# second-state/qwen3_asr_rs

Hardware: AMD Instinct MI355X
Metric: audio-seconds/sec (RTFx) Qwen3-ASR-0.6B greedy, 30s clips (higher is better)
Workload: dtype bf16; 1 GPU; Qwen3-ASR-0.6b bf16, batch=1 x 30s synthetic 16kHz clip per GPU, 100 new tokens (fixed, EOS ignored); clips_per_gpu=1, parallelism=dp1 (independent utterances per GPU, no data-path collective)

## Files before the change

### qwen3_asr_rs_amd/csrc/k_gemv.hip

```cpp
#include <algorithm>
#include <type_traits>

#include "argmax.h"


namespace q3a {

int gemv_rows_per_wave(const GemvArgs& a) {
  const int logical = (a.mode == 2) ? a.N / 2 : a.N;
  if (logical >= 32768 && a.K <= 2048) return 4;
  if (logical >= 4096 || a.mode == 2) return 2;
  return 1;
}
int gemv_blocks(const GemvArgs& a) {
  const int pr = gemv_rows_per_wave(a);
  const int rows_per_wave = (a.mode == 2) ? pr / 2 : pr;
  const int logical = (a.mode == 2) ? a.N / 2 : a.N;
  return (logical + 4 * rows_per_wave - 1) / (4 * rows_per_wave);
}

namespace {

constexpr int ATTN_F_MAX = 1024;
struct AttnTables {
// ... 90 lines not shown
    M = Mn;
  }
  const float inv = 1.0f / L;
#pragma unroll
  for (int e = 0; e < 8; ++e) x[e] *= inv;
}

template <int PR>
__device__ __forceinline__ void gemv_rows(const GemvArgs& a, int g, int (&prow)[PR]) {
#pragma unroll
  for (int i = 0; i < PR; ++i) {
    if (a.mode == 2) {
      const int j = g * (PR / 2) + (i >> 1);
      prow[i] = (j / 16) * 32 + (j % 16) + ((i & 1) ? 16 : 0);
    } else {
      prow[i] = g * PR + i;
    }
    if (prow[i] >= a.N) prow[i] = -1;
  }
}

__device__ __forceinline__ float dot8(const uint4& w, const float (&x)[8], float s) {
  f32x2_t a = f32x2_t{bf16lo(w.x), bf16hi(w.x)} * f32x2_t{x[0], x[1]};
  a += f32x2_t{bf16lo(w.y), bf16hi(w.y)} * f32x2_t{x[2], x[3]};
  a += f32x2_t{bf16lo(w.z), bf16hi(w.z)} * f32x2_t{x[4], x[5]};
  a += f32x2_t{bf16lo(w.w), bf16hi(w.w)} * f32x2_t{x[6], x[7]};
  return s + (a.x + a.y);
}

__device__ __forceinline__ uint4 ld_w16(const GemvArgs& a, int prow, int k) {
  const int row = prow >= 0 ? prow : a.N - 1;
  return ld_stream16(a.W + (size_t)row * a.K + k);
}
template <int KI, int PR>
__device__ __forceinline__ void request_rows(const GemvArgs& a, const int (&prow)[PR], const int (&kk)[KI], uint4 (&wq)[KI][PR]) {
#pragma unroll
  for (int it = 0; it < KI; ++it)
#pragma unroll
    for (int i = 0; i < PR; ++i) wq[it][i] = ld_w16(a, prow[i], kk[it]);
}
template <int KI>
__device__ __forceinline__ void lane_cols(int lane, int K, bool (&kin)[KI], int (&kk)[KI]) {
#pragma unroll
  for (int it = 0; it < KI; ++it) {
    const int k = lane * 8 + it * 512;
    kin[it] = k < K;
    kk[it] = kin[it] ? k : 0;
  }
}
template <int KI>
__device__ __forceinline__ void fetch_cols(const GemvArgs& a, const int (&kk)[KI], float4 (&xr)[KI][2], float4 (&nr)[KI][2]) {
#pragma unroll
  for (int it = 0; it < KI; ++it) {
    xr[it][0] = *reinterpret_cast<const float4*>(a.x + kk[it]);
    xr[it][1] = *reinterpret_cast<const float4*>(a.x + kk[it] + 4);
    nr[it][0] = *reinterpret_cast<const float4*>(a.rms_w + kk[it]);
    nr[it][1] = *reinterpret_cast<const float4*>(a.rms_w + kk[it] + 4);
  }
}
template <int KI, bool YY = false>
__device__ __forceinline__ void unpack_cols(int K, const bool (&kin)[KI], const float4 (&xr)[KI][2], const float4 (&nr)[KI][2],
                                            float (&x)[KI][8], float& ss, float* yy = nullptr) {
#pragma unroll
  for (int it = 0; it < KI; ++it) {
    const float4 v0 = xr[it][0], v1 = xr[it][1];
    const float xv[8] = {v0.x, v0.y, v0.z, v0.w, v1.x, v1.y, v1.z, v1.w};
#pragma unroll
    for (int e = 0; e < 8; ++e) x[it][e] = (K == KI * 512 || kin[it]) ? xv[e] : 0.f;
    const float4 w0 = nr[it][0], w1 = nr[it][1];
    const float wv[8] = {w0.x, w0.y, w0.z, w0.w, w1.x, w1.y, w1.z, w1.w};
#pragma unroll
    for (int e = 0; e < 8; ++e) { ss += x[it][e] * x[it][e]; x[it][e] *= wv[e]; }
    if constexpr (YY) {
#pragma unroll
      for (int e = 0; e < 8; ++e) *yy += x[it][e] * x[it][e];
    }
  }
}
template <bool LP, int NB>
__device__ __forceinline__ ArgmaxAcc<LP> merge_wave_partials(float (*am_v)[NB], int (*am_i)[NB], float (*am_s)[NB], int b) {
  ArgmaxAcc<LP> r{am_v[0][b], am_i[0][b], LP ? am_s[0][b] : 0.f};
  for (int w = 1; w < 4; ++w) r.merge(am_v[w][b], am_i[w][b], LP ? am_s[w][b] : 0.f);
  return r;
}

template <int NB, int PR, bool LP>
__device__ __forceinline__ void gemv_epilogue(const GemvArgs& a, int g, const int (&prow)[PR], float (&acc)[PR][NB],
                                              float (*am_v)[NB], int (*am_i)[NB], float (*am_s)[NB]) {
  const int tid = threadIdx.x, lane = tid & 63, wave = tid >> 6;
  if (a.mode == 3) {
    ArgmaxAcc<LP> m[NB];
    float lv[LP ? PR : 1][NB];
#pragma unroll
    for (int i = 0; i < PR; ++i) {
      if constexpr (LP) {
#pragma unroll
        for (int b = 0; b < NB; ++b) lv[i][b] = -INFINITY;
      }
      if (prow[i] < 0) continue;
#pragma unroll
      for (int b = 0; b < NB; ++b) {
        float v = acc[i][b];
        if (a.bias) v += a.bias[prow[i]];
        if (lane == 0 && a.out) a.out[(size_t)b * a.ldo + prow[i]] = v;
        if (v > m[b].v) { m[b].v = v; m[b].i = prow[i]; }
        if constexpr (LP) lv[i][b] = v;
      }
    }
    if (lane == 0) {
#pragma unroll
      for (int b = 0; b < NB; ++b) {
        am_v[wave][b] = m[b].v; am_i[wave][b] = m[b].i;
        if constexpr (LP) {
          float ws = 0.f;
#pragma unroll
          for (int i = 0; i < PR; ++i) ws += lse_term(1.f, lv[i][b], m[b].v);
          am_s[wave][b] = ws;
        }
      }
    }
    __syncthreads();
    if (tid < NB) merge_wave_partials<LP, NB>(am_v, am_i, am_s, tid).store(a.part, tid, g >> 2);
    return;
  }
  if (lane != 0) return;
  if (a.mode != 2) {
#pragma unroll
    for (int i = 0; i < PR; ++i) {
      if (prow[i] < 0) continue;
      const int n = prow[i];
#pragma unroll
      for (int b = 0; b < NB; ++b) {
        float v = acc[i][b];
        if (a.bias) v += a.bias[n];
        if (a.mode == 1) v += a.resid[(size_t)b * a.ldo + n];
        a.out[(size_t)b * a.ldo + n] = v;
      }
    }
  } else {
#pragma unroll
    for (int i = 0; i + 1 < PR; i += 2) {
      if (prow[i] < 0) continue;
      const int j = g * (PR / 2) + (i >> 1);
#pragma unroll
      for (int b = 0; b < NB; ++b) {
        float gv = acc[i][b], uv = acc[i + 1][b];
        if (a.bias) { gv += a.bias[prow[i]]; uv += a.bias[prow[i + 1]]; }
        a.out[(size_t)b * a.ldo + j] = silu_sel(gv, a.fast_math != 0) * uv;
      }
    }
  }
}

template <int PR, int KI, bool RMS, bool ATTN, int MF, bool XL, bool XP = false>
__device__ __forceinline__ void gemv1_body(const GemvArgs& a) {
  static_assert(!XL || !ATTN, "the merged attention vector already goes through LDS");
  static_assert(!XP || (XL && RMS), "the partial vectors are added in the hand-over of the norm-fused XL form");
  constexpr bool XH = !RMS && !ATTN && KI > 4;
  constexpr bool XLDS = XL || XH;
  static_assert(!XH || KI % 2 == 0, "the hand-over stores unguarded: its rounds of 1024 columns must end at KI * 512");
  __shared__ __attribute__((aligned(16))) float x_lds[(ATTN || XLDS) ? KI * 512 : 4], xl_w[(XL && RMS) ? KI * 512 : 4];
  const int tid = threadIdx.x, lane = tid & 63, wave = tid >> 6;
  Q3A_STAMP_ENTRY(t_entry);
  const int K = a.K;
  const int g = blockIdx.x * 4 + wave;
  int prow[PR];
  gemv_rows<PR>(a, g, prow);
  bool kin[KI];
  int kk[KI];
#pragma unroll
  for (int it = 0; it < KI; ++it) {
    const int k = lane * 8 + it * 512;
    kin[it] = k < K;
    kk[it] = kin[it] ? k : 0;
  }
  float4 xr[KI][2], nr[RMS ? KI : 1][2];
  uint4 wq[KI][PR];
  constexpr int XLN = (KI + 1) / 2;
  float4 xl_rx[XLDS ? XLN : 1], xl_rw[(XL && RMS) ? XLN : 1];
  constexpr int XPN = XP ? GEMV_X_PARTS_MAX : 1;
  float4 xp_r[XP ? XLN : 1][XPN];
  auto request_x = [&]() {
    if (ATTN) return;
    if constexpr (XLDS) {
#pragma unroll
      for (int j = 0; j < XLN; ++j) {
        const int k = (tid + j * 256) * 4, kc = k < K ? k : 0;
        xl_rx[j] = *reinterpret_cast<const float4*>(a.x + kc);
        if constexpr (XP) {
#pragma unroll
          for (int h = 0; h < XPN; ++h)
            xp_r[j][h] = *reinterpret_cast<const float4*>(a.x_parts + (size_t)(h < a.x_nparts ? h : a.x_nparts - 1) * K + kc);
        }
        if (RMS) xl_rw[j] = *reinterpret_cast<const float4*>(a.rms_w + kc);
      }
      return;
    }
#pragma unroll
    for (int it = 0; it < KI; ++it) {
      xr[it][0] = *reinterpret_cast<const float4*>(a.x + kk[it]);
      xr[it][1] = *reinterpret_cast<const float4*>(a.x + kk[it] + 4);
      if (RMS) {
        nr[it][0] = *reinterpret_cast<const float4*>(a.rms_w + kk[it]);
        nr[it][1] = *reinterpret_cast<const float4*>(a.rms_w + kk[it] + 4);
      }
    }
  };
  auto request_w = [&]() {
#pragma unroll
    for (int it = 0; it < KI; ++it)
#pragma unroll
      for (int i = 0; i < PR; ++i) {
        const int row = prow[i] >= 0 ? prow[i] : a.N - 1;
        wq[it][i] = ld_stream16(a.W + (size_t)row * K + kk[it]);
      }
  };
  constexpr int MCH = MF > 0 ? MF : 1;
  float mg_m[MCH], mg_l[MCH];
  float4 mg_o0[MCH], mg_o1[MCH];
  const int mg_k = lane * 8 + wave * 512;
  const bool mg_on = wave < KI && mg_k < K;
  if constexpr (ATTN && MF > 0) {
    const int kc = mg_k < K ? mg_k : 0;
    const int h = kc >> 7, d = kc & 127, ns = a.attn_nsplit, base = h * ns;
    typedef float __attribute__((ext_vector_type(4), aligned(4))) f4u_t;
#pragma unroll
    for (int j = 0; j < MCH; j += 4) {
      const f4u_t m4 = *reinterpret_cast<const f4u_t*>(a.attn_pm + base + j), l4 = *reinterpret_cast<const f4u_t*>(a.attn_pl + base + j);
#pragma unroll
      for (int e = 0; e < 4; ++e) {
        mg_m[j + e] = j + e < ns ? m4[e] : -INFINITY;
        mg_l[j + e] = j + e < ns ? l4[e] : 0.f;
      }
    }
#pragma unroll
    for (int j = 0; j < MCH; ++j) attn_partial_row8(a, base, j, d, mg_o0[j], mg_o1[j]);
    __builtin_amdgcn_sched_barrier(0);
  }
  if (RMS || XLDS) { request_x(); request_w(); } else { request_w(); request_x(); }
  if constexpr (ATTN && MF > 0) __builtin_amdgcn_sched_barrier(0);
  float bv[PR], rv[PR];
#pragma unroll
  for (int i = 0; i < PR; ++i) {
    const int n = prow[i] >= 0 ? prow[i] : 0;
    bv[i] = a.bias ? a.bias[n] : 0.f;
    rv[i] = a.mode == 1 ? a.resid[n] : 0.f;
  }
  __builtin_amdgcn_sched_barrier(0);
  Q3A_STAMP_AT(a.stamp, blockIdx.x, 1);
  Q3A_STAMP_PUT(a.stamp, blockIdx.x, 0, t_entry);
  Q3A_ARG(a.out); Q3A_ARG(a.fast_math);
  if (ATTN) Q3A_ARG(a.attn_fast_exp);
  if constexpr (ATTN && MF > 0) {
    if (mg_on) {
      const bool fast = a.attn_fast_exp != 0;
      float Mn = -INFINITY;
#pragma unroll
      for (int j = 0; j < MCH; ++j) Mn = fmaxf(Mn, mg_m[j]);
      float L = 0.f, v[8];
#pragma unroll
      for (int e = 0; e < 8; ++e) v[e] = 0.f;
#pragma unroll
      for (int j = 0; j < MCH; ++j) {
        const float f = fast ? __expf(mg_m[j] - Mn) : expf(mg_m[j] - Mn);
        L += mg_l[j] * f;
        v[0] += mg_o0[j].x * f; v[1] += mg_o0[j].y * f; v[2] += mg_o0[j].z * f; v[3] += mg_o0[j].w * f;
        v[4] += mg_o1[j].x * f; v[5] += mg_o1[j].y * f; v[6] += mg_o1[j].z * f; v[7] += mg_o1[j].w * f;
      }
      const float inv = 1.0f / L;
#pragma unroll
      for (int e = 0; e < 8; ++e) v[e] *= inv;
      *reinterpret_cast<float4*>(x_lds + mg_k) = make_float4(v[0], v[1], v[2], v[3]);
      *reinterpret_cast<float4*>(x_lds + mg_k + 4) = make_float4(v[4], v[5], v[6], v[7]);
    }
    __syncthreads();
  } else if constexpr (ATTN) {
    auto merge_pieces = [&](auto fast_c, auto ch_c) {
#pragma unroll
      for (int it = 0; it < KI; ++it) {
        if ((it & 3) == wave && kin[it]) {
          float v[8];
          attn_merge8_ch<decltype(fast_c)::value, decltype(ch_c)::value>(a, 0, kk[it], v);
          *reinterpret_cast<float4*>(x_lds + kk[it]) = make_float4(v[0], v[1], v[2], v[3]);
          *reinterpret_cast<float4*>(x_lds + kk[it] + 4) = make_float4(v[4], v[5], v[6], v[7]);
        }
      }
    };
    typedef std::integral_constant<int, 4> Ch4;
    typedef std::integral_constant<int, 8> Ch8;
    if (a.attn_fast_exp) {
      if (a.attn_nsplit <= 4) merge_pieces(std::true_type{}, Ch4{}); else merge_pieces(std::true_type{}, Ch8{});
    } else {
      if (a.attn_nsplit <= 4) merge_pieces(std::false_type{}, Ch4{}); else merge_pieces(std::false_type{}, Ch8{});
    }
    __syncthreads();
  }
  if constexpr (XLDS) {
#pragma unroll
    for (int j = 0; j < XLN; ++j) {
      const int k = (tid + j * 256) * 4;
      if (XH || k < KI * 512) {
        float4 v = xl_rx[j];
        if constexpr (XP) {
#pragma unroll
          for (int h = 0; h < XPN; ++h)
            if (h < a.x_nparts) { v.x += xp_r[j][h].x; v.y += xp_r[j][h].y; v.z += xp_r[j][h].z; v.w += xp_r[j][h].w; }
          if (blockIdx.x == 0 && k < K) *reinterpret_cast<float4*>(a.x_out + k) = v;
        }
        *reinterpret_cast<float4*>(x_lds + k) = make_float4(v.x, v.y, v.z, v.w);
        if (RMS) *reinterpret_cast<float4*>(xl_w + k) = xl_rw[j];
      }
    }
    __syncthreads();
  }
  if constexpr (ATTN || XLDS) {
#pragma unroll
    for (int it = 0; it < KI; ++it) {
      xr[it][0] = *reinterpret_cast<const float4*>(x_lds + kk[it]);
      xr[it][1] = *reinterpret_cast<const float4*>(x_lds + kk[it] + 4);
      if (XL && RMS) {
        nr[it][0] = *reinterpret_cast<const float4*>(xl_w + kk[it]);
        nr[it][1] = *reinterpret_cast<const float4*>(xl_w + kk[it] + 4);
      }
    }
  }
  Q3A_STAMP_AT(a.stamp, blockIdx.x, 2);
  float x[KI][8], acc[PR];
  float ss = 0.f;
#pragma unroll
  for (int it = 0; it < KI; ++it) {
    const float4 v0 = xr[it][0], v1 = xr[it][1];
    const float xv[8] = {v0.x, v0.y, v0.z, v0.w, v1.x, v1.y, v1.z, v1.w};
#pragma unroll
    for (int e = 0; e < 8; ++e) x[it][e] = (K == KI * 512 || kin[it]) ? xv[e] : 0.f;
    if (RMS) {
      const float4 w0 = nr[it][0], w1 = nr[it][1];
      const float wv[8] = {w0.x, w0.y, w0.z, w0.w, w1.x, w1.y, w1.z, w1.w};
#pragma unroll
      for (int e = 0; e < 8; ++e) { ss += x[it][e] * x[it][e]; x[it][e] *= wv[e]; }
    }
  }
#pragma unroll
  for (int i = 0; i < PR; ++i) acc[i] = 0.f;
#pragma unroll
  for (int it = 0; it < KI; ++it)
#pragma unroll
    for (int i = 0; i < PR; ++i) acc[i] = dot8(wq[it][i], x[it], acc[i]);
  if (wave == 0) asm volatile("" ::"v"(acc[0]));
  Q3A_STAMP_AT(a.stamp, blockIdx.x, 3);
  float rstd = 1.0f;
  if (RMS) rstd = rstd_of(wave_sum_fast(ss) / (float)K + a.eps, a.fast_math != 0);
#pragma unroll
  for (int i = 0; i < PR; ++i) acc[i] = wave_sum_fast(acc[i]) * rstd + bv[i];
  if (lane != 0) return;
  if (a.mode != 2) {
#pragma unroll
    for (int i = 0; i < PR; ++i)
      if (prow[i] >= 0) a.out[prow[i]] = acc[i] + rv[i];
  } else {
#pragma unroll
    for (int i = 0; i + 1 < PR; i += 2)
      if (prow[i] >= 0) a.out[g * (PR / 2) + (i >> 1)] = silu_sel(acc[i], a.fast_math != 0) * acc[i + 1];
  }
  Q3A_STAMP_AT(a.stamp, blockIdx.x, 4);
}

struct GemvTail {
  float* out; int fast_math;
  Q3A_STAMP_FIELD
};
struct GemvAttnTail {
  float* out; const float* bias; int attn_heads; int attn_fast_exp; int fast_math;
  Q3A_STAMP_FIELD
};
#ifdef Q3A_STAMP
#define Q3A_STAMP_COPY(dst, src) (dst).stamp = (src).stamp
#else
#define Q3A_STAMP_COPY(dst, src) do { } while (0)
#endif
template <int PR, int KI, bool RMS, bool ATTN, int MF = 0, bool XL = false>
__global__ __launch_bounds__(256) void gemv1_kernel(const uint16_t* W, const float* x, const float* rms_w, const float* bias,
                                                    const float* resid, int N, int K, int mode, float eps, GemvTail t) {
  static_assert(!ATTN, "the ATTN forms take the partials in their head");
  GemvArgs a{};
  a.W = W; a.x = x; a.rms_w = rms_w; a.bias = bias; a.resid = resid; a.N = N; a.K = K; a.mode = mode; a.eps = eps;
  a.out = t.out; a.fast_math = t.fast_math;
  Q3A_STAMP_COPY(a, t);
  gemv1_body<PR, KI, RMS, ATTN, MF, XL>(a);
}
template <int PR, int KI, bool RMS, bool ATTN, int MF = 0, bool XL = false>
__global__ __launch_bounds__(256) void gemv1_kernel(const float* attn_pm, const float* attn_pl, const float* attn_po, const uint16_t* W,
                                                    const float* resid, int N, int K, int attn_nsplit, int mode, GemvAttnTail t) {
  static_assert(ATTN && !RMS, "the plain forms take x and the norm weight in their head");
  GemvArgs a{};
  a.attn_pm = attn_pm; a.attn_pl = attn_pl; a.attn_po = attn_po; a.W = W; a.resid = resid; a.N = N; a.K = K; a.attn_nsplit = attn_nsplit;
  a.mode = mode;
  a.out = t.out; a.bias = t.bias; a.attn_heads = t.attn_heads; a.attn_fast_exp = t.attn_fast_exp; a.fast_math = t.fast_math;
  Q3A_STAMP_COPY(a, t);
  gemv1_body<PR, KI, RMS, ATTN, MF, XL>(a);
}

struct GemvXpTail {
  float* out; float* x_out; int fast_math;
  Q3A_STAMP_FIELD
};
template <int PR, int KI>
__global__ __launch_bounds__(256) void gemv1_xp_kernel(const uint16_t* W, const float* x, const float* rms_w, const float* x_parts,
                                                       const float* bias, int N, int K, int x_nparts, float eps, GemvXpTail t) {
  GemvArgs a{};
  a.W = W; a.x = x; a.rms_w = rms_w; a.x_parts = x_parts; a.bias = bias; a.N = N; a.K = K; a.x_nparts = x_nparts; a.eps = eps; a.mode = 2;
  a.out = t.out; a.x_out = t.x_out; a.fast_math = t.fast_math;
  Q3A_STAMP_COPY(a, t);
  gemv1_body<PR, KI, true, false, 0, true, true>(a);
}

struct OprojHeadTail {
  const float* bias;
  Q3A_STAMP_FIELD
};
template <int CW, int RB>
__global__ __launch_bounds__(256) void oproj_head_kernel(const float* pm, const float* pl, const float* po, const uint16_t* W, float* y_part,
                                                         int N, int K, int nsplit, int n_parts, OprojHeadTail t) {
  constexpr int NS = OPROJ_HEAD_MAX_SPLITS;
  constexpr int HEADS = CW / 128;
  constexpr int LPR = CW / 8;
  constexpr int RPI = 64 / LPR;
  constexpr int NI = RB / 4 / RPI;
  constexpr int E4 = CW / 4;
  constexpr int TG = 256 / E4;
  constexpr int SPT = NS / TG;
  static_assert(CW == 128 || CW == 256 || CW == 512, "a slice is 1, 2 or 4 q heads");
  static_assert(NI >= 1 && NI * RPI * 4 == RB && SPT * TG == NS && HEADS * NS <= 256, "row block / split plan");
  __shared__ float m_s[HEADS * NS], l_s[HEADS * NS], inv_s[HEADS];
  __shared__ __attribute__((aligned(16))) float red[TG][CW];
  const int tid = threadIdx.x, lane = tid & 63, wave = tid >> 6;
  Q3A_STAMP_ENTRY(t_entry);
  const int part = blockIdx.x % n_parts, rb = blockIdx.x / n_parts;
  const int q0 = part * HEADS;
  const int e4 = tid % E4, tg = tid / E4, hh = e4 >> 5, d = (e4 & 31) * 4;
  const int st = tid < HEADS * NS ? tid : HEADS * NS - 1, st_j = st % NS, st_jc = st_j < nsplit ? st_j : nsplit - 1;
  float st_m = pm[(size_t)(q0 + st / NS) * nsplit + st_jc], st_l = pl[(size_t)(q0 + st / NS) * nsplit + st_jc];
  float4 o[SPT];
#pragma unroll
  for (int i = 0; i < SPT; ++i) {
    const int j = tg + i * TG, jc = j < nsplit ? j : nsplit - 1;
    o[i] = *reinterpret_cast<const float4*>(po + ((size_t)(q0 + hh) * nsplit + jc) * 128 + d);
  }
  __builtin_amdgcn_sched_barrier(0);
  const int row0 = rb * RB + wave * (RB / 4) + lane / LPR;
  uint4 wq[NI];
#pragma unroll
  for (int i = 0; i < NI; ++i) {
    const int row = row0 + i * RPI, rc = row < N ? row : N - 1;
    wq[i] = ld_stream16(W + (size_t)rc * K + part * CW + (lane % LPR) * 8);
  }
  __builtin_amdgcn_sched_barrier(0);
  float bv[NI];
#pragma unroll
  for (int i = 0; i < NI; ++i) {
    const int row = row0 + i * RPI;
    bv[i] = (t.bias && part == 0) ? t.bias[row < N ? row : N - 1] : 0.f;
  }
  __builtin_amdgcn_sched_barrier(0);
  Q3A_STAMP_AT(t.stamp, blockIdx.x, 1);
  Q3A_STAMP_PUT(t.stamp, blockIdx.x, 0, t_entry);
  if (st_j >= nsplit) { st_m = -INFINITY; st_l = 0.f; }
  if (tid < HEADS * NS) { m_s[tid] = st_m; l_s[tid] = st_l; }
  __syncthreads();
  float M = -INFINITY, L = 0.f;
#pragma unroll
  for (int j = 0; j < NS; ++j) M = fmaxf(M, m_s[hh * NS + j]);
#pragma unroll
  for (int j = 0; j < NS; ++j) L += l_s[hh * NS + j] * __expf(m_s[hh * NS + j] - M);
  float4 acc = make_float4(0.f, 0.f, 0.f, 0.f);
#pragma unroll
  for (int i = 0; i < SPT; ++i) {
    const float f = __expf(m_s[hh * NS + tg + i * TG] - M);
    acc.x += o[i].x * f; acc.y += o[i].y * f; acc.z += o[i].z * f; acc.w += o[i].w * f;
  }
  *reinterpret_cast<float4*>(&red[tg][e4 * 4]) = acc;
  if (tg == 0 && (e4 & 31) == 0) inv_s[hh] = 1.0f / L;
  __syncthreads();
  const int c0 = (lane % LPR) * 8;
  float x[8];
#pragma unroll
  for (int e = 0; e < 8; ++e) x[e] = 0.f;
#pragma unroll
  for (int g = 0; g < TG; ++g) {
    const float4 a0 = *reinterpret_cast<const float4*>(&red[g][c0]), a1 = *reinterpret_cast<const float4*>(&red[g][c0 + 4]);
    x[0] += a0.x; x[1] += a0.y; x[2] += a0.z; x[3] += a0.w; x[4] += a1.x; x[5] += a1.y; x[6] += a1.z; x[7] += a1.w;
  }
  const float inv = inv_s[c0 >> 7];
#pragma unroll
  for (int e = 0; e < 8; ++e) x[e] *= inv;
  Q3A_STAMP_AT(t.stamp, blockIdx.x, 2);
  float y[NI];
#pragma unroll
  for (int i = 0; i < NI; ++i) {
    float v = row16_sum(dot8(wq[i], x, 0.f));
    if (LPR >= 32) v = xor16_sum(v);
    if (LPR >= 64) v = xor32_sum(v);
    y[i] = v + bv[i];
  }
  if (wave == 0) asm volatile("" ::"v"(y[0]));
  Q3A_STAMP_AT(t.stamp, blockIdx.x, 3);
  if (lane % LPR == 0) {
#pragma unroll
    for (int i = 0; i < NI; ++i) {
      const int row = row0 + i * RPI;
      if (row < N) y_part[(size_t)part * N + row] = y[i];
    }
  }
  Q3A_STAMP_AT(t.stamp, blockIdx.x, 4);
}

template <int PR, int KI, bool LP = false>
__device__ __forceinline__ void gemv1_head_block(const GemvArgs& a, int blk, float (&am_v)[4][1], int (&am_i)[4][1], float (*am_s)[1],
                                                 ArgmaxAcc<LP>& out) {
  const int tid = threadIdx.x, lane = tid & 63, wave = tid >> 6;
  const int g = blk * 4 + wave;
  int prow[PR];
  gemv_rows<PR>(a, g, prow);
  bool kin[KI];
  int kk[KI];
  lane_cols<KI>(lane, a.K, kin, kk);
  float4 xr[KI][2], nr[KI][2];
  uint4 wq[KI][PR];
  fetch_cols<KI>(a, kk, xr, nr);
  request_rows<KI, PR>(a, prow, kk, wq);
  float bv[PR];
#pragma unroll
  for (int i = 0; i < PR; ++i) bv[i] = a.bias ? a.bias[prow[i] >= 0 ? prow[i] : 0] : 0.f;
  __builtin_amdgcn_sched_barrier(0);
  float x[KI][8], acc[PR];
  float ss = 0.f;
  unpack_cols<KI>(a.K, kin, xr, nr, x, ss);
#pragma unroll
  for (int i = 0; i < PR; ++i) acc[i] = 0.f;
#pragma unroll
  for (int it = 0; it < KI; ++it)
#pragma unroll
    for (int i = 0; i < PR; ++i) acc[i] = dot8(wq[it][i], x[it], acc[i]);
  const float rstd = rstd_of(wave_sum_fast(ss) / (float)a.K + a.eps, a.fast_math != 0);
#pragma unroll
  for (int i = 0; i < PR; ++i) acc[i] = wave_sum_fast(acc[i]) * rstd + bv[i];
  ArgmaxAcc<LP> m;
#pragma unroll
  for (int i = 0; i < PR; ++i) {
    if (prow[i] < 0) continue;
    if (lane == 0 && a.out) a.out[prow[i]] = acc[i];
    if (acc[i] > m.v) { m.v = acc[i]; m.i = prow[i]; }
  }
  if (lane == 0) { am_v[wave][0] = m.v; am_i[wave][0] = m.i; }
  if constexpr (LP) {
    float ws = 0.f;
#pragma unroll
    for (int i = 0; i < PR; ++i) ws += prow[i] < 0 ? 0.f : lse_term(1.f, acc[i], m.v);
    if (lane == 0) am_s[wave][0] = ws;
  }
  __syncthreads();
  if (tid == 0) out = merge_wave_partials<LP, 1>(am_v, am_i, am_s, 0);
}

template <int PR, int KI, bool LP = false>
__global__ __launch_bounds__(256) void gemv1_head_kernel(const uint16_t* W, const float* x, const float* rms_w, const float* bias, float* out,
                                                         int N, int K, float eps, int fast_math, ArgmaxPartials part) {
// ... 184 lines not shown
    if (i < nb) t = fmaxf(t, v.x);
    if (i + 1 < nb) t = fmaxf(t, v.y);
    if (i + 2 < nb) t = fmaxf(t, v.z);
    if (i + 3 < nb) t = fmaxf(t, v.w);
  };
#pragma unroll
  for (int j = 0; j < PRE; ++j) fold(lv[j], tid + j * 256);
  for (int i4 = tid + PRE * 256; i4 < n4; i4 += 256) fold(lo4[i4], i4);
  t = wave_max(t);
  if (lane == 0) red[wave] = t;
  cand[tid] = 0;
  __syncthreads();
  const float T = fmaxf(fmaxf(red[0], red[1]), fmaxf(red[2], red[3]));
  if (mb < nb) cand[tid] = !(hv < T);
  __syncthreads();
  const int nj = (nb - blockIdx.x + G - 1) / G;
  ArgmaxAcc<false> best;
  int nc = 0;
  for (int j = 0; j < nj; ++j) {
    if (!cand[j]) continue;
    ArgmaxAcc<false> r;
    gemv1_head_block<PR, KI>(g, blockIdx.x + j * G, am_v, am_i, nullptr, r);
    if (tid == 0) best.merge(r);
    ++nc;
    __syncthreads();
  }
  if (tid == 0) {
    best.store(g.part, 0, blockIdx.x);
    if (tl.stats) {
      if (nc) atomicAdd(&tl.stats[0], nc);
      if (blockIdx.x == 0) atomicAdd(&tl.stats[1], 1);
    }
  }
}

template <int NB, int PR, int PF, bool LP = false>
__global__ __launch_bounds__(256) void gemvn_kernel(GemvArgs a) {
  extern __shared__ __attribute__((aligned(16))) float xs[];
  __shared__ float red[NB][4];
  __shared__ float am_v[4][NB];
  __shared__ int am_i[4][NB];
  __shared__ float am_s[LP ? 4 : 1][NB];
  const int tid = threadIdx.x, lane = tid & 63, wave = tid >> 6;
  const int K = a.K;
  const int g = blockIdx.x * 4 + wave;
  int prow[PR];
  gemv_rows<PR>(a, g, prow);
  bool kin[PF];
  int kk[PF];
  lane_cols<PF>(lane, K, kin, kk);
  uint4 wq[PF][PR];
  request_rows<PF, PR>(a, prow, kk, wq);
  __shared__ AttnTables f_s;
  if (a.attn_po) attn_scales(a, NB, f_s);
#pragma unroll
  for (int b = 0; b < NB; ++b) {
    float ss = 0.f;
    for (int k = tid * 8; k < K; k += 2048) {
      float x[8];
      if (a.attn_po) {
        attn_combined8(a, b, k, f_s, x);
      } else {
        const float4 v0 = *reinterpret_cast<const float4*>(a.x + (size_t)b * a.ldx + k);
        const float4 v1 = *reinterpret_cast<const float4*>(a.x + (size_t)b * a.ldx + k + 4);
        x[0] = v0.x; x[1] = v0.y; x[2] = v0.z; x[3] = v0.w; x[4] = v1.x; x[5] = v1.y; x[6] = v1.z; x[7] = v1.w;
      }
      if (a.rms_w) {
        const float4 w0 = *reinterpret_cast<const float4*>(a.rms_w + k);
        const float4 w1 = *reinterpret_cast<const float4*>(a.rms_w + k + 4);
        const float wv[8] = {w0.x, w0.y, w0.z, w0.w, w1.x, w1.y, w1.z, w1.w};
#pragma unroll
        for (int e = 0; e < 8; ++e) { ss += x[e] * x[e]; x[e] *= wv[e]; }
      }
      *reinterpret_cast<float4*>(xs + (size_t)b * K + k) = make_float4(x[0], x[1], x[2], x[3]);
      *reinterpret_cast<float4*>(xs + (size_t)b * K + k + 4) = make_float4(x[4], x[5], x[6], x[7]);
    }
    if (a.rms_w) {
      ss = wave_sum_fast(ss);
      if (lane == 0) red[b][wave] = ss;
    }
  }
  __syncthreads();
  float acc[PR][NB];
#pragma unroll
  for (int i = 0; i < PR; ++i)
#pragma unroll
    for (int b = 0; b < NB; ++b) acc[i][b] = 0.f;
  auto fma_all = [&](const uint4 (&w)[PR], int k) {
#pragma unroll
    for (int b = 0; b < NB; ++b) {
      const float4 xa = *reinterpret_cast<const float4*>(xs + (size_t)b * K + k);
      const float4 xb = *reinterpret_cast<const float4*>(xs + (size_t)b * K + k + 4);
      const float x[8] = {xa.x, xa.y, xa.z, xa.w, xb.x, xb.y, xb.z, xb.w};
#pragma unroll
      for (int i = 0; i < PR; ++i) acc[i][b] = dot8(w[i], x, acc[i][b]);
    }
  };
#pragma unroll
  for (int it = 0; it < PF; ++it)
    if (kin[it]) fma_all(wq[it], kk[it]);
  for (int k = lane * 8 + PF * 512; k < K; k += 512) {
    uint4 w[PR];
#pragma unroll
    for (int i = 0; i < PR; ++i) w[i] = ld_w16(a, prow[i], k);
    fma_all(w, k);
  }
#pragma unroll
  for (int b = 0; b < NB; ++b) {
    float rstd = 1.0f;
    if (a.rms_w) rstd = rstd_of((red[b][0] + red[b][1] + red[b][2] + red[b][3]) / (float)K + a.eps, a.fast_math != 0);
#pragma unroll
    for (int i = 0; i < PR; ++i) acc[i][b] = wave_sum_fast(acc[i][b]) * rstd;
  }
  gemv_epilogue<NB, PR, LP>(a, g, prow, acc, am_v, am_i, am_s);
}

#define GEMV_PLAIN_ARGS(a) (a).W, (a).x, (a).rms_w, (a).bias, (a).resid, (a).N, (a).K, (a).mode, (a).eps, gemv_tail(a)
#define GEMV_ATTN_ARGS(a) (a).attn_pm, (a).attn_pl, (a).attn_po, (a).W, (a).resid, (a).N, (a).K, (a).attn_nsplit, (a).mode, gemv_attn_tail(a)
#define GEMV_HEAD_ARGS(a) (a).W, (a).x, (a).rms_w, (a).bias, (a).out, (a).N, (a).K, (a).eps, (a).fast_math, (a).part
GemvTail gemv_tail(const GemvArgs& a) {
  GemvTail t{};
  t.out = a.out; t.fast_math = a.fast_math;
  Q3A_STAMP_COPY(t, a);
  return t;
}
GemvAttnTail gemv_attn_tail(const GemvArgs& a) {
  GemvAttnTail t{};
  t.out = a.out; t.bias = a.bias; t.attn_heads = a.attn_heads; t.attn_fast_exp = a.attn_fast_exp; t.fast_math = a.fast_math;
  Q3A_STAMP_COPY(t, a);
  return t;
}

template <int PR, int KI>
void launch1k(const GemvArgs& a, hipStream_t s) {
  const dim3 grid(gemv_blocks(a)), block(256);
  if (a.attn_po) {
    if constexpr (KI <= 4) {
      if (a.attn_nsplit <= 4) { hipLaunchKernelGGL((gemv1_kernel<PR, KI, false, true, 4>), grid, block, 0, s, GEMV_ATTN_ARGS(a)); return; }
      if (a.attn_nsplit <= 8) { hipLaunchKernelGGL((gemv1_kernel<PR, KI, false, true, 8>), grid, block, 0, s, GEMV_ATTN_ARGS(a)); return; }
    }
    hipLaunchKernelGGL((gemv1_kernel<PR, KI, false, true>), grid, block, 0, s, GEMV_ATTN_ARGS(a));
  } else if (a.rms_w) {
    if (a.mode == 3) {
      if (a.part.sum) hipLaunchKernelGGL((gemv1_head_kernel<PR, KI, true>), grid, block, 0, s, GEMV_HEAD_ARGS(a));
      else hipLaunchKernelGGL((gemv1_head_kernel<PR, KI>), grid, block, 0, s, GEMV_HEAD_ARGS(a));
      return;
    }
    if constexpr (KI == 2) {
      if constexpr (PR == 2) {
        if (a.x_parts) {
          GemvXpTail t{};
          t.out = a.out; t.x_out = a.x_out; t.fast_math = a.fast_math;
          Q3A_STAMP_COPY(t, a);
          hipLaunchKernelGGL((gemv1_xp_kernel<PR, KI>), grid, block, 0, s, a.W, a.x, a.rms_w, a.x_parts, a.bias, a.N, a.K, a.x_nparts, a.eps, t);
          return;
        }
      }
      hipLaunchKernelGGL((gemv1_kernel<PR, KI, true, false, 0, true>), grid, block, 0, s, GEMV_PLAIN_ARGS(a));
    } else {
      hipLaunchKernelGGL((gemv1_kernel<PR, KI, true, false>), grid, block, 0, s, GEMV_PLAIN_ARGS(a));
    }
  } else {
    hipLaunchKernelGGL((gemv1_kernel<PR, KI, false, false>), grid, block, 0, s, GEMV_PLAIN_ARGS(a));
  }
}
template <int PR>
void launch1(const GemvArgs& a, hipStream_t s) {
  if (a.K <= 1024) launch1k<PR, 2>(a, s);
  else if (a.K <= 2048) launch1k<PR, 4>(a, s);
  else if constexpr (PR < 4) {
    if (a.K <= 3072) launch1k<PR, 6>(a, s); else launch1k<PR, 12>(a, s);
  }
}
template <int NB, int PR, int PF>
void launchn(const GemvArgs& a, hipStream_t s) {
  if (a.part.sum) hipLaunchKernelGGL((gemvn_kernel<NB, PR, PF, true>), dim3(gemv_blocks(a)), dim3(256), (size_t)NB * a.K * sizeof(float), s, a);
  else hipLaunchKernelGGL((gemvn_kernel<NB, PR, PF>), dim3(gemv_blocks(a)), dim3(256), (size_t)NB * a.K * sizeof(float), s, a);
}

}

int lm_head_prune_blocks(const GemvArgs& g) { return (g.N + 15) / 16; }
const char* launch_lm_head_quantize(const uint16_t* W, int N, int K, int8_t* Q, float* qs, hipStream_t s) {
  const int cols = lm_head_q_cols(K);
  if (cols == 0 || K % 8 != 0) return "lm_head_quantize: hidden size beyond the one-sequence GEMV";
  if (hipMemsetAsync(Q, 0, (size_t)N * cols, s) != hipSuccess) return "lm_head_quantize: memset failed";
  hipLaunchKernelGGL(lm_head_quantize_kernel, dim3((N + 3) / 4), dim3(256), 0, s, W, N, K, cols, Q, qs);
  return nullptr;
}
const char* lm_head_prune_check(const LmHeadPruneArgs& a) {
  const GemvArgs& g = a.g;
  if (g.mode != 3 || !g.rms_w || !g.x || g.attn_po) return "lm_head_prune: needs the plain mode-3 GEMV with a fused norm";
  if (g.bias && !a.logit_bias) return "lm_head_prune: the only bias the bound covers is the logit bias (finite or -inf entries)";
  if (g.part.sum) return "lm_head_prune: token log-probabilities need every logit (the full GEMV)";
  if (gemv_rows_per_wave(g) != 4 || gemv_blocks(g) != lm_head_prune_blocks(g)) return "lm_head_prune: the GEMV does not run 16-row blocks here";
  if (g.K % 8 != 0 || a.qcols != lm_head_q_cols(g.K)) return "lm_head_prune: int8 row width does not match the hidden size";
  if (!a.Wq || !a.qs || !a.blk_lo || !a.blk_hi || !g.part.val) return "lm_head_prune: missing buffer";
  if (const char* e = argmax_partials_check(g.part, 1)) return e;
  return nullptr;
}
const char* launch_lm_head_approx(const LmHeadPruneArgs& a, hipStream_t s) {
  if (const char* e = lm_head_prune_check(a)) return e;
  const GemvArgs& g = a.g;
  const int n_blk = lm_head_prune_blocks(g);
  const dim3 grid((n_blk + 3) / 4), block(256);
  const double nu = (double)a.qcols * 0x1p-24;
  const LmHeadApproxTail t{g.eps, g.fast_math, (float)(nu / (1.0 - nu)) * (1.0f + 0x1p-20f), a.blk_lo, a.blk_hi, a.dbg};
#define LM_HEAD_APPROX_ARGS a.Wq, g.x, g.rms_w, a.qs, g.bias, g.N, g.K, a.qcols, n_blk, t
  if (a.g.bias) {
    if (a.qcols == 1024) hipLaunchKernelGGL(lm_head_approx_bias_kernel<2>, grid, block, 0, s, LM_HEAD_APPROX_ARGS);
    else hipLaunchKernelGGL(lm_head_approx_bias_kernel<4>, grid, block, 0, s, LM_HEAD_APPROX_ARGS);
  } else {
    if (a.qcols == 1024) hipLaunchKernelGGL(lm_head_approx_kernel<2>, grid, block, 0, s, LM_HEAD_APPROX_ARGS);
    else hipLaunchKernelGGL(lm_head_approx_kernel<4>, grid, block, 0, s, LM_HEAD_APPROX_ARGS);
  }
#undef LM_HEAD_APPROX_ARGS
  return nullptr;
}
int lm_head_rescore_groups(const GemvArgs& g, int n_cu) {
  const int nb = lm_head_prune_blocks(g);
  return std::min(nb, std::max(n_cu > 0 ? n_cu : 256, (nb + 255) / 256));
}
const char* launch_lm_head_rescore(const LmHeadPruneArgs& a, int groups, hipStream_t s) {
  if (const char* e = lm_head_prune_check(a)) return e;
  const GemvArgs& g = a.g;
  const int n_blk = lm_head_prune_blocks(g);
  if (groups < 1 || groups > g.part.stride || (n_blk + groups - 1) / groups > 256) return "lm_head_prune: bad rescore grid";
  const LmHeadRescoreTail t{g.bias, g.out, g.fast_math, g.part, a.stats};
#define LM_HEAD_RESCORE_ARGS a.blk_lo, a.blk_hi, g.W, g.x, g.rms_w, n_blk, g.N, g.K, g.eps, t
  if (a.qcols == 1024) hipLaunchKernelGGL((lm_head_rescore_kernel<4, 2>), dim3(groups), dim3(256), 0, s, LM_HEAD_RESCORE_ARGS);
  else hipLaunchKernelGGL((lm_head_rescore_kernel<4, 4>), dim3(groups), dim3(256), 0, s, LM_HEAD_RESCORE_ARGS);
#undef LM_HEAD_RESCORE_ARGS
  return nullptr;
}

const char* oproj_head_check(const OprojHeadArgs& a) {
  if (!a.pm || !a.pl || !a.po || !a.W || !a.y_part || a.N < 1) return "oproj_head: missing buffer";
  if (a.N > 1024) return "oproj_head: N <= 1024 (the gate / up form that adds the partial vectors exists at K <= 1024)";
  if (a.nsplit < 1 || a.nsplit > OPROJ_HEAD_MAX_SPLITS) return "oproj_head: 1 .. 16 key splits (more: the merging o_proj of launch_gemv)";
  if (a.n_parts < 1 || a.K != a.n_parts * 512) return "oproj_head: a slice is 512 columns (two kv heads of two q heads)";
  return nullptr;
}
const char* launch_oproj_head(const OprojHeadArgs& a, hipStream_t s) {
  if (const char* e = oproj_head_check(a)) return e;
  OprojHeadTail t{};
  t.bias = a.bias;
  Q3A_STAMP_COPY(t, a);
  constexpr int rb = 16;
  const dim3 grid(a.n_parts * ((a.N + rb - 1) / rb)), block(256);
#define OPROJ_HEAD_ARGS a.pm, a.pl, a.po, a.W, a.y_part, a.N, a.K, a.nsplit, a.n_parts, t
  hipLaunchKernelGGL((oproj_head_kernel<512, rb>), grid, block, 0, s, OPROJ_HEAD_ARGS);
#undef OPROJ_HEAD_ARGS
  return nullptr;
}

const char* launch_gemv(const GemvArgs& a0, int NB, hipStream_t s) {
  if (a0.K % 8 != 0) return "gemv: K must be a multiple of 8";
  if (a0.K > 6144) return "gemv: K > 6144 unsupported";
  if (a0.mode == 2 && a0.N % 32 != 0) return "gemv: GLU needs N % 32 == 0";
  if (a0.mode == 3 && !a0.rms_w) return "gemv: mode 3 (the lm_head) needs the fused final norm";
  if (a0.mode == 3 && !a0.part.val) return "gemv: argmax partial buffer missing";
  if (const char* e = argmax_partials_check(a0.part, a0.mode == 3 ? gemv_blocks(a0) : 0)) return e;
  if (a0.part.sum && a0.mode != 3) return "gemv: log-sum partials need mode 3";
  if (a0.attn_po && (a0.K % 128 != 0 || a0.K != a0.attn_heads * 128)) return "gemv: attention-partial input needs K = heads*128";
  if (a0.attn_po && a0.rms_w) return "gemv: attention-partial input cannot be combined with a fused RMSNorm";
  if (a0.attn_po && (NB < 4 ? NB : 4) * a0.attn_heads * a0.attn_nsplit > ATTN_F_MAX) return "gemv: too many attention splits for the LDS scale table";
  if (a0.x_parts && (NB != 1 || !a0.x || !a0.rms_w || a0.mode != 2 || a0.K > 1024 || a0.x_nparts < 1 || a0.x_nparts > GEMV_X_PARTS_MAX || !a0.x_out))
    return "gemv: partial vectors are added in the one-sequence norm-fused GLU form at K <= 1024 only (1 .. 4 vectors, x_out set)";
  const int pr = gemv_rows_per_wave(a0);
  const int nb_cap = (int)((64 * 1024) / ((size_t)a0.K * 4));
  int done = 0;
  while (done < NB) {
    GemvArgs a = a0;
    if (a0.x) a.x = a0.x + (size_t)done * a0.ldx;
    if (a0.out) a.out = a0.out + (size_t)done * a0.ldo;
    if (a0.resid) a.resid = a0.resid + (size_t)done * a0.ldo;
    a.part = a0.part.at(done);
    if (a0.attn_po) {
      const size_t adv = (size_t)done * a0.attn_heads * a0.attn_nsplit;
      a.attn_pm = a0.attn_pm + adv; a.attn_pl = a0.attn_pl + adv; a.attn_po = a0.attn_po + adv * 128;
    }
    int nb = NB - done;
    if (nb >= 4 && nb_cap >= 4) nb = 4;
    else if (nb >= 2 && nb_cap >= 2) nb = 2;
    else nb = 1;
    if (nb == 1) {
      if (pr == 4) launch1<4>(a, s); else if (pr == 2) launch1<2>(a, s); else launch1<1>(a, s);
    } else if (nb == 2) {
      if (pr == 4) launchn<2, 4, 2>(a, s); else if (pr == 2) launchn<2, 2, 4>(a, s); else launchn<2, 1, 6>(a, s);
    } else {
      if (pr == 4) launchn<4, 4, 2>(a, s); else if (pr == 2) launchn<4, 2, 4>(a, s); else launchn<4, 1, 6>(a, s);
    }
    done += nb;
  }
  return nullptr;
}

}
```

Baseline: 523.5 audio-seconds/sec.

## Split xp GEMV into wave roles with 12-wave blocks for vector handover

Replaces the norm-fused, partial-sum GEMV (gate/up with SiLU) path with a dedicated kernel using 12 waves per block. The first four waves load x and the partial vectors, the next four load the norm weight, and all waves stream weights and compute one row pair each. The aim is to spread the per-thread hand-over loads across waves so fewer registers and serial loads sit ahead of the weight stream, and to use larger blocks so fewer blocks are launched. The cost is a bigger block of 768 threads, which may lower occupancy and makes every wave wait at a block-wide barrier.

```diff
diff --git a/qwen3_asr_rs_amd/csrc/k_gemv.hip b/qwen3_asr_rs_amd/csrc/k_gemv.hip
--- a/qwen3_asr_rs_amd/csrc/k_gemv.hip
+++ b/qwen3_asr_rs_amd/csrc/k_gemv.hip
@@ -266,10 +266,9 @@
   }
 }
 
-template <int PR, int KI, bool RMS, bool ATTN, int MF, bool XL, bool XP = false>
+template <int PR, int KI, bool RMS, bool ATTN, int MF, bool XL>
 __device__ __forceinline__ void gemv1_body(const GemvArgs& a) {
   static_assert(!XL || !ATTN, "the merged attention vector already goes through LDS");
-  static_assert(!XP || (XL && RMS), "the partial vectors are added in the hand-over of the norm-fused XL form");
   constexpr bool XH = !RMS && !ATTN && KI > 4;
   constexpr bool XLDS = XL || XH;
   static_assert(!XH || KI % 2 == 0, "the hand-over stores unguarded: its rounds of 1024 columns must end at KI * 512");
@@ -292,8 +291,6 @@
   uint4 wq[KI][PR];
   constexpr int XLN = (KI + 1) / 2;
   float4 xl_rx[XLDS ? XLN : 1], xl_rw[(XL && RMS) ? XLN : 1];
-  constexpr int XPN = XP ? GEMV_X_PARTS_MAX : 1;
-  float4 xp_r[XP ? XLN : 1][XPN];
   auto request_x = [&]() {
     if (ATTN) return;
     if constexpr (XLDS) {
@@ -301,11 +298,6 @@
       for (int j = 0; j < XLN; ++j) {
         const int k = (tid + j * 256) * 4, kc = k < K ? k : 0;
         xl_rx[j] = *reinterpret_cast<const float4*>(a.x + kc);
-        if constexpr (XP) {
-#pragma unroll
-          for (int h = 0; h < XPN; ++h)
-            xp_r[j][h] = *reinterpret_cast<const float4*>(a.x_parts + (size_t)(h < a.x_nparts ? h : a.x_nparts - 1) * K + kc);
-        }
         if (RMS) xl_rw[j] = *reinterpret_cast<const float4*>(a.rms_w + kc);
       }
       return;
@@ -415,12 +407,6 @@
       const int k = (tid + j * 256) * 4;
       if (XH || k < KI * 512) {
         float4 v = xl_rx[j];
-        if constexpr (XP) {
-#pragma unroll
-          for (int h = 0; h < XPN; ++h)
-            if (h < a.x_nparts) { v.x += xp_r[j][h].x; v.y += xp_r[j][h].y; v.z += xp_r[j][h].z; v.w += xp_r[j][h].w; }
-          if (blockIdx.x == 0 && k < K) *reinterpret_cast<float4*>(a.x_out + k) = v;
-        }
         *reinterpret_cast<float4*>(x_lds + k) = make_float4(v.x, v.y, v.z, v.w);
         if (RMS) *reinterpret_cast<float4*>(xl_w + k) = xl_rw[j];
       }
@@ -514,18 +500,117 @@
   gemv1_body<PR, KI, RMS, ATTN, MF, XL>(a);
 }
 
+template <int PR, int KI, int NW, int ROLE>
+__device__ __forceinline__ void gemv1_xp_role(const GemvArgs& a, float* x_lds, float* xl_w) {
+  const int tid = threadIdx.x, lane = tid & 63, wave = tid >> 6;
+  Q3A_STAMP_ENTRY(t_entry);
+  const int K = a.K;
+  const int g = blockIdx.x * NW + wave;
+  int prow[PR];
+  gemv_rows<PR>(a, g, prow);
+  bool kin[KI];
+  int kk[KI];
+#pragma unroll
+  for (int it = 0; it < KI; ++it) {
+    const int k = lane * 8 + it * 512;
+    kin[it] = k < K;
+    kk[it] = kin[it] ? k : 0;
+  }
+  float4 xr[KI][2], nr[KI][2];
+  uint4 wq[KI][PR];
+  const int hk = (tid & (KI * 128 - 1)) * 4, hkc = hk < K ? hk : 0;
+  float4 hx, hp[GEMV_X_PARTS_MAX], hw;
+  if constexpr (ROLE == 0) {
+    hx = *reinterpret_cast<const float4*>(a.x + hkc);
+#pragma unroll
+    for (int h = 0; h < GEMV_X_PARTS_MAX; ++h)
+      hp[h] = *reinterpret_cast<const float4*>(a.x_parts + (size_t)(h < a.x_nparts ? h : a.x_nparts - 1) * K + hkc);
+  }
+  if constexpr (ROLE == 1) hw = *reinterpret_cast<const float4*>(a.rms_w + hkc);
+#pragma unroll
+  for (int it = 0; it < KI; ++it)
+#pragma unroll
+    for (int i = 0; i < PR; ++i) {
+      const int row = prow[i] >= 0 ? prow[i] : a.N - 1;
+      wq[it][i] = ld_stream16(a.W + (size_t)row * K + kk[it]);
+    }
+  float bv[PR];
+#pragma unroll
+  for (int i = 0; i < PR; ++i) bv[i] = a.bias ? a.bias[prow[i] >= 0 ? prow[i] : 0] : 0.f;
+  __builtin_amdgcn_sched_barrier(0);
+  Q3A_STAMP_AT(a.stamp, blockIdx.x, 1);
+  Q3A_STAMP_PUT(a.stamp, blockIdx.x, 0, t_entry);
+  Q3A_ARG(a.out); Q3A_ARG(a.x_out); Q3A_ARG(a.fast_math);
+  if constexpr (ROLE == 0) {
+    float4 v = hx;
+#pragma unroll
+    for (int h = 0; h < GEMV_X_PARTS_MAX; ++h)
+      if (h < a.x_nparts) { v.x += hp[h].x; v.y += hp[h].y; v.z += hp[h].z; v.w += hp[h].w; }
+    if (blockIdx.x == 0 && hk < K) *reinterpret_cast<float4*>(a.x_out + hk) = v;
+    *reinterpret_cast<float4*>(x_lds + hk) = make_float4(v.x, v.y, v.z, v.w);
+  }
+  if constexpr (ROLE == 1) *reinterpret_cast<float4*>(xl_w + hk) = make_float4(hw.x, hw.y, hw.z, hw.w);
+  __syncthreads();
+#pragma unroll
+  for (int it = 0; it < KI; ++it) {
+    xr[it][0] = *reinterpret_cast<const float4*>(x_lds + kk[it]);
+    xr[it][1] = *reinterpret_cast<const float4*>(x_lds + kk[it] + 4);
+    nr[it][0] = *reinterpret_cast<const float4*>(xl_w + kk[it]);
+    nr[it][1] = *reinterpret_cast<const float4*>(xl_w + kk[it] + 4);
+  }
+  Q3A_STAMP_AT(a.stamp, blockIdx.x, 2);
+  float x[KI][8], acc[PR];
+  float ss = 0.f;
+#pragma unroll
+  for (int it = 0; it < KI; ++it) {
+    const float4 v0 = xr[it][0], v1 = xr[it][1];
+    const float xv[8] = {v0.x, v0.y, v0.z, v0.w, v1.x, v1.y, v1.z, v1.w};
+#pragma unroll
+    for (int e = 0; e < 8; ++e) x[it][e] = (K == KI * 512 || kin[it]) ? xv[e] : 0.f;
+    const float4 w0 = nr[it][0], w1 = nr[it][1];
+    const float wv[8] = {w0.x, w0.y, w0.z, w0.w, w1.x, w1.y, w1.z, w1.w};
+#pragma unroll
+    for (int e = 0; e < 8; ++e) { ss += x[it][e] * x[it][e]; x[it][e] *= wv[e]; }
+  }
+#pragma unroll
+  for (int i = 0; i < PR; ++i) acc[i] = 0.f;
+#pragma unroll
+  for (int it = 0; it < KI; ++it)
+#pragma unroll
+    for (int i = 0; i < PR; ++i) acc[i] = dot8(wq[it][i], x[it], acc[i]);
+  if (wave == 0) asm volatile("" ::"v"(acc[0]));
+  Q3A_STAMP_AT(a.stamp, blockIdx.x, 3);
+  const float rstd = rstd_of(wave_sum_fast(ss) / (float)K + a.eps, a.fast_math != 0);
+#pragma unroll
+  for (int i = 0; i < PR; ++i) acc[i] = wave_sum_fast(acc[i]) * rstd + bv[i];
+  if (lane != 0) return;
+#pragma unroll
+  for (int i = 0; i + 1 < PR; i += 2)
+    if (prow[i] >= 0) a.out[g * (PR / 2) + (i >> 1)] = silu_sel(acc[i], a.fast_math != 0) * acc[i + 1];
+  Q3A_STAMP_AT(a.stamp, blockIdx.x, 4);
+}
+template <int PR, int KI, int NW>
+__device__ __forceinline__ void gemv1_xp_body(const GemvArgs& a) {
+  static_assert(KI == 2 && NW >= 8, "four waves own the KI * 128 sixteen-byte pieces of a vector; four more fetch the norm weight");
+  __shared__ __attribute__((aligned(16))) float x_lds[KI * 512], xl_w[KI * 512];
+  const int wave = __builtin_amdgcn_readfirstlane(threadIdx.x >> 6);
+  if (wave < 4) gemv1_xp_role<PR, KI, NW, 0>(a, x_lds, xl_w);
+  else if (wave < 8) gemv1_xp_role<PR, KI, NW, 1>(a, x_lds, xl_w);
+  else gemv1_xp_role<PR, KI, NW, 2>(a, x_lds, xl_w);
+}
 struct GemvXpTail {
   float* out; float* x_out; int fast_math;
   Q3A_STAMP_FIELD
 };
-template <int PR, int KI>
-__global__ __launch_bounds__(256) void gemv1_xp_kernel(const uint16_t* W, const float* x, const float* rms_w, const float* x_parts,
-                                                       const float* bias, int N, int K, int x_nparts, float eps, GemvXpTail t) {
+constexpr int GEMV_XP_WAVES = 12;
+template <int PR, int KI, int NW>
+__global__ __launch_bounds__(NW * 64) void gemv1_xp_kernel(const uint16_t* W, const float* x, const float* rms_w, const float* x_parts,
+                                                           const float* bias, int N, int K, int x_nparts, float eps, GemvXpTail t) {
   GemvArgs a{};
   a.W = W; a.x = x; a.rms_w = rms_w; a.x_parts = x_parts; a.bias = bias; a.N = N; a.K = K; a.x_nparts = x_nparts; a.eps = eps; a.mode = 2;
   a.out = t.out; a.x_out = t.x_out; a.fast_math = t.fast_math;
   Q3A_STAMP_COPY(a, t);
-  gemv1_body<PR, KI, true, false, 0, true, true>(a);
+  gemv1_xp_body<PR, KI, NW>(a);
 }
 
 struct OprojHeadTail {
@@ -1016,7 +1101,9 @@
           GemvXpTail t{};
           t.out = a.out; t.x_out = a.x_out; t.fast_math = a.fast_math;
           Q3A_STAMP_COPY(t, a);
-          hipLaunchKernelGGL((gemv1_xp_kernel<PR, KI>), grid, block, 0, s, a.W, a.x, a.rms_w, a.x_parts, a.bias, a.N, a.K, a.x_nparts, a.eps, t);
+          const dim3 xp_grid((a.N / 2 + GEMV_XP_WAVES - 1) / GEMV_XP_WAVES), xp_block(GEMV_XP_WAVES * 64);
+                    hipLaunchKernelGGL((gemv1_xp_kernel<PR, KI, GEMV_XP_WAVES>), xp_grid, xp_block, 0, s, a.W, a.x, a.rms_w, a.x_parts, a.bias, a.N, a.K, a.x_nparts,
+                             a.eps, t);
           return;
         }
       }
```

Result: faster. 530.0 audio-seconds/sec, median of 6 (+1.2%).
